# argumentcomputer/lurk-beta

Measured on NVIDIA H100. Metric: Lurk iterations proved/sec (fib rc=100, Nova IVC), higher is better.
Workload: dtype u32x8 (254-bit Montgomery integers)

## Files before the change

lurk-beta_b200/csrc/foldctx_impl.cuh:

```cuda
#pragma once
#include "msm_impl.cuh"
#include "poseidon_api.h"
#include "trie.cuh"
#include "spmv3.cuh"

#include <memory>
#include <string>

namespace lurk {

static constexpr int FOLD_MAX_WORLD = 16;
static constexpr int FOLD_MAX_DEPTH = 4;
static constexpr int FOLD_MAX_SPANS = 4;
static constexpr int FOLD_RO_RATE = 24;
static constexpr int FOLD_W_WINDOW = 16;
static constexpr int FOLD_T_WINDOW = 16;

template <class F>
__global__ void __launch_bounds__(256) cross_term_dev_kernel(const F *__restrict__ az1, const F *__restrict__ bz1, const F *__restrict__ cz1,
                                                             const F *__restrict__ az2, const F *__restrict__ bz2, const F *__restrict__ cz2,
                                                             const F *__restrict__ u1p, const F *__restrict__ u2p, size_t n, F *__restrict__ t) {
    const F u1 = load_fe<F>(u1p), u2 = load_fe<F>(u2p);
    for (size_t i = (size_t)blockIdx.x * blockDim.x + threadIdx.x; i < n; i += (size_t)gridDim.x * blockDim.x) {
        WideAcc<typename F::Params> acc;
        acc.clear();
        acc.mul_acc(load_fe<F>(az1 + i), load_fe<F>(bz2 + i));
        acc.mul_acc(load_fe<F>(az2 + i), load_fe<F>(bz1 + i));
        F pos = acc.reduce();
        WideAcc<typename F::Params> neg;
        neg.clear();
        neg.mul_acc(u1, load_fe<F>(cz2 + i));
        neg.mul_acc(u2, load_fe<F>(cz1 + i));
        store_fe(t + i, pos - neg.reduce());
    }
}

template <class F>
struct FoldAxpyArgs {
    F *dst[5];
    const F *src[5];
    size_t end[5];
};
template <class F>
__global__ void __launch_bounds__(256) fold_axpy_kernel(FoldAxpyArgs<F> a, const F *__restrict__ rp) {
    const F r = load_fe<F>(rp);
    const size_t total = a.end[4];
    for (size_t i = (size_t)blockIdx.x * blockDim.x + threadIdx.x; i < total; i += (size_t)gridDim.x * blockDim.x) {
        int v = 0;
        while (i >= a.end[v]) v++;
        const size_t j = v ? i - a.end[v - 1] : i;
        store_fe(a.dst[v] + j, load_fe<F>(a.dst[v] + j) + r * load_fe<F>(a.src[v] + j));
    }
}

template <class F>
__global__ void __launch_bounds__(256) span_to_mont_kernel(F *base, uint64_t first, uint64_t row_elems, uint64_t stride, uint64_t rows) {
    const uint64_t total = row_elems * rows;
    for (uint64_t i = (uint64_t)blockIdx.x * blockDim.x + threadIdx.x; i < total; i += (uint64_t)gridDim.x * blockDim.x) {
        F *p = base + first + (i / row_elems) * stride + (i % row_elems);
        store_fe(p, F::from_canonical(load_fe<F>(p)));
    }
// ... 357 lines not shown
```

lurk-beta_b200/csrc/foldctx_inst.cu:

```cuda
#include "foldctx_impl.cuh"
#include "sha256.cuh"

#include <cuda.h>
#include <cstring>

namespace lurk {
LURK_MSM_EXTERN(LURK_C)
#define LURK_FOLD_POSEIDON_EXTERN(F)                                                                          \
    extern template int launch_poseidon<F, true>(int, const void *, size_t, void *, int, int, cudaStream_t, const uint64_t *, const PoseidonGather *); \
    extern template int poseidon_instance_info<F>(int, const PoseidonParams<F> **, PoseidonLayout *);        \
    extern template int launch_bitdecomp<F>(const void *, size_t, void *, int, int, cudaStream_t, const uint64_t *); \
    extern template size_t sha256_block_len<F>(int);                                                          \
    extern template int launch_sha256_witness<F>(const void *, size_t, int, void *, const uint64_t *, int, int, cudaStream_t); \
    extern template size_t trie_block_len<F>(int, int);                                                       \
    extern template int launch_trie_witness<F>(int, int, const void *, size_t, void *, const uint64_t *, int, int, cudaStream_t);
LURK_FOLD_POSEIDON_EXTERN(Fe<Bn254Fr>)
LURK_FOLD_POSEIDON_EXTERN(Fe<Bn254Fq>)
LURK_FOLD_POSEIDON_EXTERN(Fe<PallasFq>)
LURK_FOLD_POSEIDON_EXTERN(Fe<PallasFp>)

static inline int fold_grid(size_t n, int block, int per_sm) {
    size_t want = (n + block - 1) / block;
    size_t cap = (size_t)sm_count() * per_sm;
    return (int)(want < cap ? (want ? want : 1) : cap);
// ... 11 lines not shown
}

template <class C>
struct FoldCtx final : FoldCtxBase {
    using Fb = typename C::Base;
    using Fs = typename C::Scalar;
    using Pt = XYZZ<Fb>;
    using Rec = FoldRecord<Fb, Fs>;

    FoldConfigHost cfg;
    int field_id = 0;
    size_t nz = 0;
    int D = 2;
    lurk_msm_ctx *ckW[FOLD_MAX_DEPTH] = {nullptr, nullptr, nullptr, nullptr};
    lurk_msm_ctx *ckT = nullptr, *ckChk = nullptr, *ckChkW = nullptr, *ckWbase = nullptr;
    DevBuf z1, e1, T, mv1[3], z2[FOLD_MAX_DEPTH], mv2[FOLD_MAX_DEPTH][3];
    DevBuf csr_rp[3], csr_col[3], csr_val[3];
    CsrDev csr[3];
    DevBuf ro_img, step_consts[FOLD_MAX_DEPTH], r_dev, seq_dev, rec_dev[FOLD_MAX_DEPTH + 1], run_pts, xchg, bad_dev, dummy_w, dummy_p;
    bool dummy_ready = false;
    Rec *h_rec[FOLD_MAX_DEPTH + 1] = {nullptr, nullptr, nullptr, nullptr, nullptr};
    void *h_glue[FOLD_MAX_DEPTH] = {nullptr, nullptr, nullptr, nullptr};
    void *h_x2[FOLD_MAX_DEPTH] = {nullptr, nullptr, nullptr, nullptr};
    void *h_ro[FOLD_MAX_DEPTH] = {nullptr, nullptr, nullptr, nullptr};
    size_t glue_elems = 0;
    std::vector<std::unique_ptr<FoldSlotBatch>> batches;
    std::vector<FoldSpan> spans;
    PoseidonLayout roL{};
    Fb io_tag;
    int n_absorb = 0, challenge_bits = 128;
    unsigned char kinds[FOLD_RO_RATE];
    XchgBuf<Fb> *peers[FOLD_MAX_WORLD];
    bool peers_open[FOLD_MAX_WORLD];
    bool peers_set = false;
    cudaStream_t sH = nullptr, sK[3] = {nullptr, nullptr, nullptr}, sA = nullptr, sB = nullptr, sC = nullptr, sT = nullptr;
    bool partitioned = false;
    cudaEvent_t ev_h2d[FOLD_MAX_DEPTH], ev_slot[FOLD_MAX_DEPTH][3], ev_cw[FOLD_MAX_DEPTH], ev_A[FOLD_MAX_DEPTH], ev_fold[FOLD_MAX_DEPTH],
        ev_chal[FOLD_MAX_DEPTH + 1], ev_done[FOLD_MAX_DEPTH + 1];
    bool fold_recorded[FOLD_MAX_DEPTH] = {false, false, false, false};
    bool a_recorded[FOLD_MAX_DEPTH] = {false, false, false, false};
    bool b_pending[FOLD_MAX_DEPTH + 1] = {false, false, false, false, false};
    bool running_set = false;
    bool mv1_valid = false;
    unsigned launches_a = 0, launches_b = 0;
    int device = 0;
    void *green[2] = {nullptr, nullptr};
    int partition_sms[2] = {0, 0};

    FoldCtx() {
        for (int p = 0; p < FOLD_MAX_WORLD; p++) { peers[p] = nullptr; peers_open[p] = false; }
        for (int b = 0; b < FOLD_MAX_DEPTH; b++) {
            ev_h2d[b] = ev_cw[b] = ev_A[b] = ev_fold[b] = nullptr;
            for (int k = 0; k < 3; k++) ev_slot[b][k] = nullptr;
        }
        for (int b = 0; b <= FOLD_MAX_DEPTH; b++) ev_chal[b] = ev_done[b] = nullptr;
        memset(kinds, 0, sizeof kinds);
    }

    ~FoldCtx() override {
        cudaDeviceSynchronize();
        for (int p = 0; p < FOLD_MAX_WORLD; p++)
            if (peers_open[p]) cudaIpcCloseMemHandle(peers[p]);
        for (int b = 0; b < FOLD_MAX_DEPTH; b++) {
            if (ckW[b]) lurk_msm_ctx_destroy(ckW[b]);
            if (h_glue[b]) cudaFreeHost(h_glue[b]);
            if (h_x2[b]) cudaFreeHost(h_x2[b]);
            if (h_ro[b]) cudaFreeHost(h_ro[b]);
            for (cudaEvent_t e : {ev_h2d[b], ev_cw[b], ev_A[b], ev_fold[b], ev_slot[b][0], ev_slot[b][1], ev_slot[b][2]})
                if (e) cudaEventDestroy(e);
        }
        for (int b = 0; b <= FOLD_MAX_DEPTH; b++) {
            if (h_rec[b]) cudaFreeHost(h_rec[b]);
            if (ev_chal[b]) cudaEventDestroy(ev_chal[b]);
            if (ev_done[b]) cudaEventDestroy(ev_done[b]);
        }
        if (ckT) lurk_msm_ctx_destroy(ckT);
        if (ckChk) lurk_msm_ctx_destroy(ckChk);
        if (ckChkW) lurk_msm_ctx_destroy(ckChkW);
        if (ckWbase) lurk_msm_ctx_destroy(ckWbase);
        for (auto &sb : batches)
            for (int b = 0; b < FOLD_MAX_DEPTH; b++)
                if (sb->h_pre[b]) cudaFreeHost(sb->h_pre[b]);
        for (cudaStream_t s : {sH, sK[0], sK[1], sK[2], sA, sB, sC, partitioned ? sT : (cudaStream_t) nullptr})
            if (s) cudaStreamDestroy(s);
        green_destroy();
    }

    template <class Fn>
    static bool drv(const char *name, Fn *out) {
        void *p = nullptr;
        cudaDriverEntryPointQueryResult q;
        if (cudaGetDriverEntryPoint(name, &p, cudaEnableDefault, &q) != cudaSuccess || q != cudaDriverEntryPointSuccess || !p) {
            cudaGetLastError();
            return false;
        }
        *out = reinterpret_cast<Fn>(p);
        return true;
    }
    void green_destroy() {
        typedef CUresult (*destroy_t)(CUgreenCtx);
        destroy_t fn = nullptr;
        if ((green[0] || green[1]) && drv("cuGreenCtxDestroy", &fn))
            for (void *g : green)
                if (g) fn((CUgreenCtx)g);
        green[0] = green[1] = nullptr;
    }
    int green_streams(int tiny_sms, cudaStream_t *tiny, int n_tiny, cudaStream_t *big_hi, cudaStream_t *big_lo, int n_lo) {
        typedef CUresult (*get_res_t)(CUdevice, CUdevResource *, CUdevResourceType);
        typedef CUresult (*split_t)(CUdevResource *, unsigned *, const CUdevResource *, CUdevResource *, unsigned, unsigned);
        typedef CUresult (*gen_desc_t)(CUdevResourceDesc *, CUdevResource *, unsigned);
        typedef CUresult (*green_create_t)(CUgreenCtx *, CUdevResourceDesc, CUdevice, unsigned);
        typedef CUresult (*green_stream_t)(CUstream *, CUgreenCtx, unsigned, int);
        get_res_t get_res; split_t split; gen_desc_t gen_desc; green_create_t green_create; green_stream_t green_stream;
        if (!drv("cuDeviceGetDevResource", &get_res) || !drv("cuDevSmResourceSplitByCount", &split) ||
            !drv("cuDevResourceGenerateDesc", &gen_desc) || !drv("cuGreenCtxCreate", &green_create) ||
            !drv("cuGreenCtxStreamCreate", &green_stream))
            return LURK_ERR_CUDA;
        CUdevResource all, part, rest;
        if (get_res((CUdevice)device, &all, CU_DEV_RESOURCE_TYPE_SM)) return LURK_ERR_CUDA;
        unsigned groups = 1;
        if (split(&part, &groups, &all, &rest, 0, (unsigned)tiny_sms) || groups != 1) return LURK_ERR_CUDA;
        CUdevResourceDesc desc[2] = {nullptr, nullptr};
        if (gen_desc(&desc[0], &part, 1) || gen_desc(&desc[1], &rest, 1)) return LURK_ERR_CUDA;
        if (green_create((CUgreenCtx *)&green[0], desc[0], (CUdevice)device, CU_GREEN_CTX_DEFAULT_STREAM) ||
            green_create((CUgreenCtx *)&green[1], desc[1], (CUdevice)device, CU_GREEN_CTX_DEFAULT_STREAM)) { green_destroy(); return LURK_ERR_CUDA; }
        partition_sms[0] = (int)part.sm.smCount;
        partition_sms[1] = (int)rest.sm.smCount;
        int rc = 0;
        for (int k = 0; k < n_tiny; k++) rc |= green_stream((CUstream *)(tiny + k), (CUgreenCtx)green[0], CU_STREAM_NON_BLOCKING, -1);
        rc |= green_stream((CUstream *)big_hi, (CUgreenCtx)green[1], CU_STREAM_NON_BLOCKING, -1);
        for (int k = 0; k < n_lo; k++) rc |= green_stream((CUstream *)(big_lo + k), (CUgreenCtx)green[1], CU_STREAM_NON_BLOCKING, 0);
        if (rc) { green_destroy(); return LURK_ERR_CUDA; }
        return LURK_OK;
    }

    int init(const FoldConfigHost &c, const uint64_t *const row_ptr[3], const uint32_t *const col[3], const uint8_t *const val[3], int fmt,
             lurk_msm_ctx *ck_w, lurk_msm_ctx *ck_t) override {
        cfg = c;
        D = c.depth;
        nz = (size_t)c.n_w + 1 + (size_t)c.n_x;
        field_id = C::ID == 0 ? LURK_FIELD_BN254_FR : C::ID == 1 ? LURK_FIELD_BN254_FQ : C::ID == 2 ? LURK_FIELD_PALLAS_FQ : LURK_FIELD_PALLAS_FP;
        LURK_CUDA_TRY(cudaGetDevice(&device));
        if (ck_w->curve_id != C::ID || ck_t->curve_id != C::ID) { set_error("commitment key belongs to another curve"); return LURK_ERR_ARG; }
        if (ck_w->n < c.n_w || ck_t->n < c.n_rows) { set_error("commitment key shorter than the witness / the constraint count"); return LURK_ERR_ARG; }
        if (ck_w->device != device || ck_t->device != device) { set_error("commitment key lives on another device"); return LURK_ERR_ARG; }
// ... 20 lines not shown
                ckT->n = c.n_rows;
                ckT->d_table = nullptr;
                ckT->owns_table = false;
                ckT->fixed_c = 0;
                LURK_TRY(msm_precompute<C>(ckT, want));
            }
        }
        LURK_TRY(lurk_msm_ctx_clone(ck_t, &ckChk));
        LURK_TRY(lurk_msm_ctx_clone(ck_w, &ckChkW));
        for (int b = 0; b < D; b++) lurk_msm_ctx_set_profiling(ckW[b], 1);
        lurk_msm_ctx_set_profiling(ckT, 1);

        int lo = 0, hi = 0;
        LURK_CUDA_TRY(cudaDeviceGetStreamPriorityRange(&lo, &hi));
        if (c.latency_sms > 0) {
            cudaStream_t tiny[2] = {nullptr, nullptr}, big_lo[4] = {nullptr, nullptr, nullptr, nullptr};
            if (green_streams(c.latency_sms, tiny, 2, &sB, big_lo, 4) != LURK_OK) {
                set_error("SM partitioning (green contexts) is not available on this driver");
                return LURK_ERR_CUDA;
            }
            sT = tiny[0]; sC = tiny[1];
            sK[0] = big_lo[0]; sK[1] = big_lo[1]; sK[2] = big_lo[2]; sA = big_lo[3];
            partitioned = true;
        } else {
            LURK_CUDA_TRY(cudaStreamCreateWithPriority(&sB, cudaStreamNonBlocking, hi));
            for (int k = 0; k < 3; k++) LURK_CUDA_TRY(cudaStreamCreateWithPriority(&sK[k], cudaStreamNonBlocking, lo));
            LURK_CUDA_TRY(cudaStreamCreateWithPriority(&sA, cudaStreamNonBlocking, lo));
            LURK_CUDA_TRY(cudaStreamCreateWithPriority(&sC, cudaStreamNonBlocking, lo));
            sT = sB;
        }
        LURK_CUDA_TRY(cudaStreamCreateWithPriority(&sH, cudaStreamNonBlocking, lo));
        if (partitioned) {
            for (lurk_msm_ctx *m : {ckW[0], ckW[1], ckW[2], ckW[3], ckT, ckChk, ckChkW}) {
                if (!m) continue;
                m->tiny_stream = sT;
                LURK_CUDA_TRY(cudaEventCreateWithFlags(&m->ev_fork, cudaEventDisableTiming));
                LURK_CUDA_TRY(cudaEventCreateWithFlags(&m->ev_join, cudaEventDisableTiming));
            }
        }
        auto mkev = [](cudaEvent_t *e) { return cudaEventCreateWithFlags(e, cudaEventDisableTiming); };
        for (int b = 0; b < D; b++) {
            LURK_CUDA_TRY(mkev(&ev_h2d[b])); LURK_CUDA_TRY(mkev(&ev_cw[b])); LURK_CUDA_TRY(mkev(&ev_A[b])); LURK_CUDA_TRY(mkev(&ev_fold[b]));
            for (int k = 0; k < 3; k++) LURK_CUDA_TRY(mkev(&ev_slot[b][k]));
        }
        for (int b = 0; b <= D; b++) { LURK_CUDA_TRY(mkev(&ev_chal[b])); LURK_CUDA_TRY(mkev(&ev_done[b])); }

        LURK_TRY(z1.alloc(nz * sizeof(Fs)));
        LURK_TRY(e1.alloc((size_t)c.n_rows * sizeof(Fs)));
        LURK_TRY(T.alloc((size_t)c.n_rows * sizeof(Fs)));
        for (int m = 0; m < 3; m++) LURK_TRY(mv1[m].alloc((size_t)c.n_rows * sizeof(Fs)));
        const Fs one = Fs::one();
        for (int b = 0; b < D; b++) {
            LURK_TRY(z2[b].alloc(nz * sizeof(Fs)));
            LURK_CUDA_TRY(cudaMemset(z2[b].p, 0, nz * sizeof(Fs)));
            LURK_CUDA_TRY(cudaMemcpy(z2[b].as<Fs>() + c.n_w, &one, sizeof(Fs), cudaMemcpyHostToDevice));
            for (int m = 0; m < 3; m++) LURK_TRY(mv2[b][m].alloc((size_t)c.n_rows * sizeof(Fs)));
            LURK_TRY(step_consts[b].alloc(FOLD_RO_RATE * sizeof(Fb)));
            LURK_CUDA_TRY(cudaMemset(step_consts[b].p, 0, FOLD_RO_RATE * sizeof(Fb)));
            LURK_CUDA_TRY(cudaMallocHost(&h_ro[b], FOLD_RO_RATE * 32));
            memset(h_ro[b], 0, FOLD_RO_RATE * 32);
            if (c.n_x) { LURK_CUDA_TRY(cudaMallocHost(&h_x2[b], (size_t)c.n_x * 32)); memset(h_x2[b], 0, (size_t)c.n_x * 32); }
        }
        LURK_CUDA_TRY(cudaMemset(z1.p, 0, nz * sizeof(Fs)));
        LURK_CUDA_TRY(cudaMemset(e1.p, 0, (size_t)c.n_rows * sizeof(Fs)));
        for (int b = 0; b <= D; b++) {
            LURK_TRY(rec_dev[b].alloc(sizeof(Rec)));
            LURK_CUDA_TRY(cudaMemset(rec_dev[b].p, 0, sizeof(Rec)));
            LURK_CUDA_TRY(cudaMallocHost((void **)&h_rec[b], sizeof(Rec)));
            memset(h_rec[b], 0, sizeof(Rec));
        }
        LURK_TRY(r_dev.alloc(sizeof(Fs)));
        LURK_TRY(seq_dev.alloc(sizeof(unsigned long long)));
        LURK_CUDA_TRY(cudaMemset(seq_dev.p, 0, sizeof(unsigned long long)));
        LURK_TRY(run_pts.alloc(2 * sizeof(Pt)));
        LURK_CUDA_TRY(cudaMemset(run_pts.p, 0, 2 * sizeof(Pt)));
        LURK_TRY(bad_dev.alloc(sizeof(SatCount)));
        LURK_TRY(xchg.alloc(sizeof(XchgBuf<Fb>)));
        LURK_CUDA_TRY(cudaMemset(xchg.p, 0, sizeof(XchgBuf<Fb>)));
        peers[c.rank] = xchg.as<XchgBuf<Fb>>();

        for (int m = 0; m < 3; m++) {
            const size_t nnz = c.n_rows ? (size_t)row_ptr[m][c.n_rows] : 0;
            for (size_t k = 0; k < nnz; k++)
                if (col[m][k] >= nz) { set_error("matrix %d: column %u out of range", m, col[m][k]); return LURK_ERR_ARG; }
            LURK_TRY(csr_rp[m].alloc(((size_t)c.n_rows + 1) * sizeof(uint64_t)));
            LURK_TRY(csr_col[m].alloc(std::max<size_t>(1, nnz) * sizeof(uint32_t)));
// ... 124 lines not shown
        else if (which == FOLD_BUF_RO) { p = h_ro[b]; n = FOLD_RO_RATE * 32; }
        else { set_error("no host buffer %d", which); return LURK_ERR_ARG; }
        if (ptr) *ptr = p;
        if (bytes) *bytes = n;
        return LURK_OK;
    }
    int device_buffer(int b, int which, void **ptr, size_t *bytes) override {
        void *p = nullptr;
        size_t n = 0;
        if (which >= 0) {
            LURK_TRY(chk_b(b));
            if (which >= (int)batches.size()) { set_error("no slot batch %d", which); return LURK_ERR_ARG; }
            p = batches[which]->d_pre[b].p; n = batches[which]->bytes();
        } else if (which == FOLD_BUF_W2) { LURK_TRY(chk_b(b)); p = z2[b].p; n = nz * 32; }
        else if (which == FOLD_BUF_RO) { LURK_TRY(chk_b(b)); p = step_consts[b].p; n = FOLD_RO_RATE * 32; }
        else if (which == FOLD_BUF_T) { p = T.p; n = (size_t)cfg.n_rows * 32; }
        else if (which == FOLD_BUF_Z1) { p = z1.p; n = nz * 32; }
        else if (which == FOLD_BUF_E1) { p = e1.p; n = (size_t)cfg.n_rows * 32; }
        else { set_error("no device buffer %d", which); return LURK_ERR_ARG; }
        if (ptr) *ptr = p;
        if (bytes) *bytes = n;
        return LURK_OK;
    }

    int exchange_handle(uint8_t out[64]) override {
        static_assert(sizeof(cudaIpcMemHandle_t) == 64, "handle size");
        cudaIpcMemHandle_t h;
        LURK_CUDA_TRY(cudaIpcGetMemHandle(&h, xchg.p));
        memcpy(out, &h, 64);
        return LURK_OK;
    }
    int set_peers(const uint8_t *handles) override {
        if (cfg.world <= 1) return LURK_OK;
// ... 28 lines not shown
        *out = Pt::from_affine(a);
        return LURK_OK;
    }

    int upload_vec(void *dst, const uint8_t *src, size_t n, int fmt) {
        if (!n) return LURK_OK;
        LURK_CUDA_TRY(cudaMemcpyAsync(dst, src, n * 32, cudaMemcpyHostToDevice, sB));
        int bad = 0;
        LURK_TRY(check_reduced_dev<Fs>(dst, n, sB, &bad));
        if (bad) { set_error("%d element(s) not reduced below the field modulus", bad); return LURK_ERR_RANGE; }
        if (fmt == LURK_FMT_CANONICAL) LURK_TRY(convert_dev<Fs>(dst, n, LURK_FMT_MONTGOMERY, dst, sB));
        return LURK_OK;
    }
    int set_running(const uint8_t *w, const uint8_t *e, const uint8_t *u, const uint8_t *x, const uint8_t *comm_w, const uint8_t *comm_e,
                    int fmt) override {
        LURK_TRY(sync());
        LURK_TRY(upload_vec(z1.p, w, cfg.n_w, fmt));
        LURK_TRY(upload_vec(z1.as<Fs>() + cfg.n_w, u, 1, fmt));
        LURK_TRY(upload_vec(z1.as<Fs>() + cfg.n_w + 1, x, cfg.n_x, fmt));
        LURK_TRY(upload_vec(e1.p, e, cfg.n_rows, fmt));
        Pt pts[2];
        LURK_TRY(point_from_bytes(comm_w, fmt, &pts[0]));
        LURK_TRY(point_from_bytes(comm_e, fmt, &pts[1]));
        LURK_CUDA_TRY(cudaMemcpyAsync(run_pts.p, pts, sizeof pts, cudaMemcpyHostToDevice, sB));
        LURK_CUDA_TRY(cudaStreamSynchronize(sB));
        running_set = true;
        mv1_valid = false;
        return LURK_OK;
    }
    int download_vec(uint8_t *dst, const void *src, size_t n, int fmt) {
        if (!n || !dst) return LURK_OK;
        if (fmt == LURK_FMT_MONTGOMERY) {
            LURK_CUDA_TRY(cudaMemcpyAsync(dst, src, n * 32, cudaMemcpyDeviceToHost, sB));
        } else {
            void *tmp = nullptr;
            LURK_CUDA_TRY(cudaMallocAsync(&tmp, n * 32, sB));
            int rc = convert_dev<Fs>(src, n, LURK_FMT_CANONICAL, tmp, sB);
            cudaError_t e = cudaMemcpyAsync(dst, tmp, n * 32, cudaMemcpyDeviceToHost, sB);
            cudaFreeAsync(tmp, sB);
            LURK_TRY(rc);
            LURK_CUDA_TRY(e);
        }
        return LURK_OK;
    }
    int get_running(uint8_t *w, uint8_t *e, uint8_t *u, uint8_t *x, uint8_t *comm_w, uint8_t *comm_e, int fmt) override {
        LURK_TRY(sync());
        LURK_TRY(download_vec(w, z1.p, cfg.n_w, fmt));
        LURK_TRY(download_vec(u, z1.as<Fs>() + cfg.n_w, 1, fmt));
        LURK_TRY(download_vec(x, z1.as<Fs>() + cfg.n_w + 1, cfg.n_x, fmt));
        LURK_TRY(download_vec(e, e1.p, cfg.n_rows, fmt));
        Pt pts[2];
        LURK_CUDA_TRY(cudaMemcpyAsync(pts, run_pts.p, sizeof pts, cudaMemcpyDeviceToHost, sB));
        LURK_CUDA_TRY(cudaStreamSynchronize(sB));
        if (comm_w) point_to_bytes(pts[0], fmt, comm_w);
        if (comm_e) point_to_bytes(pts[1], fmt, comm_e);
        return LURK_OK;
    }

    int prepare_dummy() {
        if (dummy_ready) return LURK_OK;
// ... 29 lines not shown
        LURK_TRY(dummy_p.alloc(64));
        LURK_CUDA_TRY(cudaMemcpy(dummy_p.p, pt, 64, cudaMemcpyHostToDevice));
        for (int k = 0; k < D; k++) { ckW[k]->d_sub = dummy_w.p; ckW[k]->d_offset = dummy_p.p; }
        return LURK_OK;
    }

    int stage_a(int b, int flags, int fmt) override {
        LURK_TRY(chk_b(b));
        LURK_TRY(prepare_dummy());
        if (fmt != LURK_FMT_CANONICAL && fmt != LURK_FMT_MONTGOMERY) { set_error("bad format %d", fmt); return LURK_ERR_ARG; }
        if (b_pending[b]) { set_error("buffer %d: the previous step's result has not been collected", b); return LURK_ERR_ARG; }
        const bool staged = !(flags & FOLD_INPUTS_RESIDENT);
        static const bool skip_a = getenv("LURK_FOLD_SKIP_STAGE_A") != nullptr;
        if (skip_a && !staged && a_recorded[b]) return LURK_OK;
        if (!staged && fmt != LURK_FMT_MONTGOMERY) { set_error("device-resident inputs are Montgomery form"); return LURK_ERR_ARG; }
        Fs *W2 = z2[b].as<Fs>();
        unsigned k = 0;
        if (fold_recorded[b]) LURK_CUDA_TRY(cudaStreamWaitEvent(sH, ev_fold[b], 0));
        if (staged) {
            for (auto &sb : batches)
                if (sb->count) LURK_CUDA_TRY(cudaMemcpyAsync(sb->d_pre[b].p, sb->h_pre[b], sb->bytes(), cudaMemcpyHostToDevice, sH));
            size_t off = 0;
            for (const FoldSpan &s : spans) {
                LURK_CUDA_TRY(cudaMemcpy2DAsync(W2 + s.first, s.stride * 32, (const uint8_t *)h_glue[b] + off * 32, s.row_elems * 32, s.row_elems * 32,
                                                s.rows, cudaMemcpyHostToDevice, sH));
                if (fmt == LURK_FMT_CANONICAL) {
                    span_to_mont_kernel<Fs><<<fold_grid(s.rows * s.row_elems, 256, 4), 256, 0, sH>>>(W2, s.first, s.row_elems, s.stride, s.rows);
                    k++;
                }
                off += s.rows * s.row_elems;
            }
            if (cfg.n_x) {
                LURK_CUDA_TRY(cudaMemcpyAsync(W2 + cfg.n_w + 1, h_x2[b], (size_t)cfg.n_x * 32, cudaMemcpyHostToDevice, sH));
// ... 19 lines not shown
            } else if (sb->arity) {
                LURK_TRY((launch_poseidon<Fs, true>(sb->arity, sb->d_pre[b].p, sb->count, W2, fmt, LURK_FMT_MONTGOMERY, st, sb->d_offsets.as<uint64_t>())));
            } else {
                uint32_t mod[8];
                for (int i = 0; i < 8; i++) mod[i] = Fs::Params::MOD(i);
                LURK_TRY(bitdecomp_fold(sb->d_pre[b].p, sb->count, W2, bitdecomp_block_host(mod), fmt, st, sb->d_offsets.as<uint64_t>()));
            }
            k++;
        }
        for (int s = 0; s < 3; s++) LURK_CUDA_TRY(cudaEventRecord(ev_slot[b][s], sK[s]));
        for (int s = 1; s < 3; s++) LURK_CUDA_TRY(cudaStreamWaitEvent(sK[0], ev_slot[b][s], 0));
        LURK_TRY(msm_launch<C>(ckW[b], W2, cfg.n_w, LURK_FMT_MONTGOMERY, sK[0], false));
        k += ckW[b]->last_launches;
        LURK_CUDA_TRY(cudaEventRecord(ev_cw[b], partitioned ? sT : sK[0]));
        for (int s = 0; s < 3; s++) LURK_CUDA_TRY(cudaStreamWaitEvent(sA, ev_slot[b][s], 0));
        if (cfg.n_rows) {
            spmv3_kernel<Fs><<<dim3(fold_grid(cfg.n_rows, 256, 8), 3), 256, 0, sA>>>(csr[0], csr[1], csr[2], cfg.n_rows, z2[b].as<Fs>(), mv2[b][0].as<Fs>(),
                                                                                    mv2[b][1].as<Fs>(), mv2[b][2].as<Fs>());
            k++;
        }
        LURK_CUDA_TRY(cudaGetLastError());
        LURK_CUDA_TRY(cudaEventRecord(ev_A[b], sA));
        a_recorded[b] = true;
        launches_a = k;
        return LURK_OK;
    }

    int bitdecomp_fold(const void *d_vals, size_t n, void *d_base, int blk, int fmt, cudaStream_t st, const uint64_t *d_offs) {
        if (fmt == LURK_FMT_MONTGOMERY) return launch_bitdecomp<Fs>(d_vals, n, d_base, blk, LURK_FMT_MONTGOMERY, st, d_offs);
        LURK_TRY(convert_dev<Fs>(d_vals, n, LURK_FMT_MONTGOMERY, const_cast<void *>(d_vals), st));
// ... 16 lines not shown
        a.mode = mode;
        a.r_out = r_dev.as<Fs>();
        a.rec = rec_dev[rec_index].as<Rec>();
        return a;
    }
    int need_peers() const {
        if (cfg.world > 1 && !peers_set) { set_error("sharded key: call lurk_fold_ctx_set_peers before the first step"); return LURK_ERR_ARG; }
        return LURK_OK;
    }

    int init_running(int b) override {
        LURK_TRY(chk_b(b));
        LURK_TRY(need_peers());
        if (!a_recorded[b]) { set_error("buffer %d: stage A has not been enqueued", b); return LURK_ERR_ARG; }
        if (b_pending[b]) { set_error("buffer %d: result not collected", b); return LURK_ERR_ARG; }
        LURK_CUDA_TRY(cudaStreamWaitEvent(sB, ev_A[b], 0));
        LURK_CUDA_TRY(cudaMemcpyAsync(z1.p, z2[b].p, nz * sizeof(Fs), cudaMemcpyDeviceToDevice, sB));
        LURK_CUDA_TRY(cudaMemsetAsync(e1.p, 0, (size_t)cfg.n_rows * sizeof(Fs), sB));
        for (int m = 0; m < 3 && cfg.n_rows; m++)
            LURK_CUDA_TRY(cudaMemcpyAsync(mv1[m].p, mv2[b][m].p, (size_t)cfg.n_rows * sizeof(Fs), cudaMemcpyDeviceToDevice, sB));
        mv1_valid = true;
        LURK_CUDA_TRY(cudaStreamWaitEvent(sT, ev_cw[b], 0));
        fold_challenge_kernel<C><<<1, 64, 0, sT>>>(challenge_args(ckW[b]->scratch.result.template as<Pt>(), nullptr, b, b, FOLD_MODE_COMMIT_ONLY));
        LURK_CUDA_TRY(cudaGetLastError());
        LURK_CUDA_TRY(cudaEventRecord(ev_chal[b], sT));
        if (sT != sB) LURK_CUDA_TRY(cudaStreamWaitEvent(sB, ev_chal[b], 0));
        LURK_CUDA_TRY(cudaEventRecord(ev_fold[b], sB));
        fold_recorded[b] = true;
        LURK_CUDA_TRY(cudaStreamWaitEvent(sC, ev_chal[b], 0));
        fold_commitments_kernel<C><<<1, 64, 0, sC>>>(run_pts.as<Pt>(), run_pts.as<Pt>() + 1, rec_dev[b].as<Rec>(), 1);
        LURK_CUDA_TRY(cudaGetLastError());
        LURK_CUDA_TRY(cudaMemcpyAsync(h_rec[b], rec_dev[b].p, sizeof(Rec), cudaMemcpyDeviceToHost, sC));
        LURK_CUDA_TRY(cudaEventRecord(ev_done[b], sC));
        b_pending[b] = true;
        running_set = true;
        launches_b = 2;
        return LURK_OK;
    }

    int stage_b_launch(int b) override {
        LURK_TRY(chk_b(b));
        LURK_TRY(need_peers());
        if (!running_set) { set_error("no running instance (lurk_fold_ctx_init_running or _set_running first)"); return LURK_ERR_ARG; }
        if (!a_recorded[b]) { set_error("buffer %d: stage A has not been enqueued", b); return LURK_ERR_ARG; }
        if (b_pending[b]) { set_error("buffer %d: the previous step's result has not been collected", b); return LURK_ERR_ARG; }
        unsigned k = 0;
        const size_t rows = cfg.n_rows;
        if (rows && !mv1_valid) {
            spmv3_kernel<Fs><<<dim3(fold_grid(rows, 256, 8), 3), 256, 0, sB>>>(csr[0], csr[1], csr[2], rows, z1.as<Fs>(), mv1[0].as<Fs>(), mv1[1].as<Fs>(),
                                                                             mv1[2].as<Fs>());
            k++;
        }
        mv1_valid = true;
        LURK_CUDA_TRY(cudaStreamWaitEvent(sB, ev_A[b], 0));
        if (rows) {
            cross_term_dev_kernel<Fs><<<fold_grid(rows, 256, 8), 256, 0, sB>>>(mv1[0].as<Fs>(), mv1[1].as<Fs>(), mv1[2].as<Fs>(), mv2[b][0].as<Fs>(),
                                                                              mv2[b][1].as<Fs>(), mv2[b][2].as<Fs>(), z1.as<Fs>() + cfg.n_w,
                                                                              z2[b].as<Fs>() + cfg.n_w, rows, T.as<Fs>());
            k++;
        }
        LURK_TRY(msm_launch<C>(ckT, T.p, rows, LURK_FMT_MONTGOMERY, sB, false));
        k += rows ? ckT->last_launches : 0;
        if (sT != sB && !rows) {
            LURK_CUDA_TRY(cudaEventRecord(ev_chal[b], sB));
            LURK_CUDA_TRY(cudaStreamWaitEvent(sT, ev_chal[b], 0));
        }
        LURK_CUDA_TRY(cudaStreamWaitEvent(sT, ev_cw[b], 0));
        fold_challenge_kernel<C><<<1, 64, 0, sT>>>(challenge_args(ckW[b]->scratch.result.template as<Pt>(), ckT->scratch.result.template as<Pt>(), b, b,
                                                                  FOLD_MODE_FOLD));
        k++;
        LURK_CUDA_TRY(cudaEventRecord(ev_chal[b], sT));
        if (sT != sB) LURK_CUDA_TRY(cudaStreamWaitEvent(sB, ev_chal[b], 0));
        {
            FoldAxpyArgs<Fs> ax;
            ax.dst[0] = z1.as<Fs>(); ax.src[0] = z2[b].as<Fs>(); ax.end[0] = nz;
            ax.dst[1] = e1.as<Fs>(); ax.src[1] = T.as<Fs>(); ax.end[1] = nz + rows;
            for (int m = 0; m < 3; m++) { ax.dst[2 + m] = mv1[m].as<Fs>(); ax.src[2 + m] = mv2[b][m].as<Fs>(); ax.end[2 + m] = nz + (size_t)(2 + m) * rows; }
            fold_axpy_kernel<Fs><<<fold_grid(ax.end[4], 256, 8), 256, 0, sB>>>(ax, r_dev.as<Fs>());
            k++;
        }
        LURK_CUDA_TRY(cudaGetLastError());
        LURK_CUDA_TRY(cudaEventRecord(ev_fold[b], sB));
        fold_recorded[b] = true;
        LURK_CUDA_TRY(cudaStreamWaitEvent(sC, ev_chal[b], 0));
        fold_commitments_kernel<C><<<1, 64, 0, sC>>>(run_pts.as<Pt>(), run_pts.as<Pt>() + 1, rec_dev[b].as<Rec>(), 0);
        k++;
        LURK_CUDA_TRY(cudaGetLastError());
        LURK_CUDA_TRY(cudaMemcpyAsync(h_rec[b], rec_dev[b].p, sizeof(Rec), cudaMemcpyDeviceToHost, sC));
        LURK_CUDA_TRY(cudaEventRecord(ev_done[b], sC));
        b_pending[b] = true;
        launches_b = k;
        return LURK_OK;
    }

    int collect(int b, FoldResultHost *out, int fmt) override {
        LURK_TRY(chk_b(b));
        if (!b_pending[b]) { set_error("buffer %d: nothing to collect", b); return LURK_ERR_ARG; }
        LURK_CUDA_TRY(cudaEventSynchronize(ev_done[b]));
        b_pending[b] = false;
        const Rec &r = *h_rec[b];
        if (out) {
            point_bytes(r.cw_x, r.cw_y, r.cw_inf, fmt, out->comm_w);
            point_bytes(r.ct_x, r.ct_y, r.ct_inf, fmt, out->comm_t);
            point_bytes(r.uw_x, r.uw_y, r.uw_inf, fmt, out->run_comm_w);
            point_bytes(r.ue_x, r.ue_y, r.ue_inf, fmt, out->run_comm_e);
            Fs rr = fmt == LURK_FMT_CANONICAL ? r.r.to_canonical() : r.r;
            memcpy(out->r, rr.v, 32);
            Fb hh = fmt == LURK_FMT_CANONICAL ? r.hash.to_canonical() : r.hash;
            memcpy(out->hash, hh.v, 32);
            out->status = (int)r.status;
            out->seq = r.seq;
        }
        if (r.status) { set_error("partial-commitment exchange timed out (a peer rank did not reach step %llu)", r.seq); return LURK_ERR_CUDA; }
        return LURK_OK;
    }

    int check_running(unsigned long long *bad_rows, int *comm_w_ok, int *comm_e_ok) override {
        LURK_TRY(need_peers());
        LURK_TRY(sync());
        const size_t rows = cfg.n_rows;
        const Fs *kept[3] = {mv1[0].as<Fs>(), mv1[1].as<Fs>(), mv1[2].as<Fs>()};
        SatCount cnt{0, 0};
        LURK_TRY(r1cs_sat_launch<Fs>(csr, rows, z1.as<Fs>(), cfg.n_w, e1.as<Fs>(), mv1_valid ? kept : nullptr, bad_dev.as<SatCount>(), sB));
        LURK_CUDA_TRY(cudaMemcpyAsync(&cnt, bad_dev.p, sizeof cnt, cudaMemcpyDeviceToHost, sB));
        LURK_TRY(msm_launch<C>(ckChkW, z1.p, cfg.n_w, LURK_FMT_MONTGOMERY, sB, false));
        LURK_TRY(msm_launch<C>(ckChk, e1.p, rows, LURK_FMT_MONTGOMERY, sB, false));
        if (sT != sB) {
            LURK_CUDA_TRY(cudaEventRecord(ev_chal[D], sB));
            LURK_CUDA_TRY(cudaStreamWaitEvent(sT, ev_chal[D], 0));
        }
        fold_challenge_kernel<C><<<1, 64, 0, sT>>>(challenge_args(ckChkW->scratch.result.template as<Pt>(), ckChk->scratch.result.template as<Pt>(), 0, D,
                                                                  FOLD_MODE_COMMIT_ONLY));
        LURK_CUDA_TRY(cudaGetLastError());
// ... 15 lines not shown
        return LURK_OK;
    }

    int stats(unsigned *la, unsigned *lb, float *acc_w_ms, float *acc_t_ms) override {
        LURK_TRY(sync());
        if (la) *la = launches_a;
        if (lb) *lb = launches_b;
        float ms = 0.f;
        if (acc_w_ms) { *acc_w_ms = 0.f; if (ckW[0]->ev0 && cudaEventElapsedTime(&ms, ckW[0]->ev0, ckW[0]->ev1) == cudaSuccess) *acc_w_ms = ms; }
        if (acc_t_ms) { *acc_t_ms = 0.f; if (ckT->ev0 && cudaEventElapsedTime(&ms, ckT->ev0, ckT->ev1) == cudaSuccess) *acc_t_ms = ms; }
        cudaGetLastError();
        return LURK_OK;
    }

    int sync() override {
        for (cudaStream_t s : {sH, sK[0], sK[1], sK[2], sA, sB, sC, sT})
            if (s) LURK_CUDA_TRY(cudaStreamSynchronize(s));
        return LURK_OK;
    }
};

template <class C>
FoldCtxBase *make_fold_ctx() { return new FoldCtx<C>(); }
template FoldCtxBase *make_fold_ctx<LURK_C>();

}
```

Baseline: 25610.

## Defer mv1 fold into next cross-term kernel and move W/E fold to side stream

The running-instance fold of the three matrix-vector products (mv1 += r*mv2) is deferred and fused into the next step's cross-term kernel, which folds, stores and consumes them in one pass. u1 is carried through a small device ring. The remaining W/E axpy now runs on a new high-priority stream sW, off the critical sB path. T is double-buffered per depth slot so the next cross term can overlap. This saves a full read/write pass over mv1 and shortens the serial chain, at the cost of more complex event dependencies and flush calls on every API path that reads state.

```diff
diff --git a/lurk-beta_b200/csrc/foldctx_impl.cuh b/lurk-beta_b200/csrc/foldctx_impl.cuh
--- a/lurk-beta_b200/csrc/foldctx_impl.cuh
+++ b/lurk-beta_b200/csrc/foldctx_impl.cuh
@@ -17,21 +17,48 @@
 static constexpr int FOLD_T_WINDOW = 16;
 
 template <class F>
-__global__ void __launch_bounds__(256) cross_term_dev_kernel(const F *__restrict__ az1, const F *__restrict__ bz1, const F *__restrict__ cz1,
-                                                             const F *__restrict__ az2, const F *__restrict__ bz2, const F *__restrict__ cz2,
-                                                             const F *__restrict__ u1p, const F *__restrict__ u2p, size_t n, F *__restrict__ t) {
-    const F u1 = load_fe<F>(u1p), u2 = load_fe<F>(u2p);
-    for (size_t i = (size_t)blockIdx.x * blockDim.x + threadIdx.x; i < n; i += (size_t)gridDim.x * blockDim.x) {
+struct CrossTermArgs {
+    F *mv1[3];
+    const F *mvp[3];
+    const F *mv2[3];
+    const F *r;
+    const F *u1, *u2;
+    F *u_next;
+    size_t n;
+    F *t;
+};
+template <class F, bool FOLD>
+__global__ void __launch_bounds__(256, 3) cross_term_fold_kernel(CrossTermArgs<F> a) {
+    F u1 = load_fe<F>(a.u1), r = F::zero();
+    if (FOLD) {
+        r = load_fe<F>(a.r);
+        u1 = u1 + r * load_fe<F>(a.u1 + 1);
+    }
+    const F u2 = load_fe<F>(a.u2);
+    if (blockIdx.x == 0 && threadIdx.x == 0) { store_fe(a.u_next, u1); store_fe(a.u_next + 1, u2); }
+    for (size_t i = (size_t)blockIdx.x * blockDim.x + threadIdx.x; i < a.n; i += (size_t)gridDim.x * blockDim.x) {
         WideAcc<typename F::Params> acc;
         acc.clear();
-        acc.mul_acc(load_fe<F>(az1 + i), load_fe<F>(bz2 + i));
-        acc.mul_acc(load_fe<F>(az2 + i), load_fe<F>(bz1 + i));
-        F pos = acc.reduce();
+        {
+            F az1 = load_fe<F>(a.mv1[0] + i);
+            if (FOLD) { az1 = az1 + r * load_fe<F>(a.mvp[0] + i); store_fe(a.mv1[0] + i, az1); }
+            acc.mul_acc(az1, load_fe<F>(a.mv2[1] + i));
+        }
+        {
+            F bz1 = load_fe<F>(a.mv1[1] + i);
+            if (FOLD) { bz1 = bz1 + r * load_fe<F>(a.mvp[1] + i); store_fe(a.mv1[1] + i, bz1); }
+            acc.mul_acc(load_fe<F>(a.mv2[0] + i), bz1);
+        }
+        const F pos = acc.reduce();
         WideAcc<typename F::Params> neg;
         neg.clear();
-        neg.mul_acc(u1, load_fe<F>(cz2 + i));
-        neg.mul_acc(u2, load_fe<F>(cz1 + i));
-        store_fe(t + i, pos - neg.reduce());
+        neg.mul_acc(u1, load_fe<F>(a.mv2[2] + i));
+        {
+            F cz1 = load_fe<F>(a.mv1[2] + i);
+            if (FOLD) { cz1 = cz1 + r * load_fe<F>(a.mvp[2] + i); store_fe(a.mv1[2] + i, cz1); }
+            neg.mul_acc(u2, cz1);
+        }
+        store_fe(a.t + i, pos - neg.reduce());
     }
 }
 
@@ -40,11 +67,12 @@
     F *dst[5];
     const F *src[5];
     size_t end[5];
+    int nv;
 };
 template <class F>
 __global__ void __launch_bounds__(256) fold_axpy_kernel(FoldAxpyArgs<F> a, const F *__restrict__ rp) {
     const F r = load_fe<F>(rp);
-    const size_t total = a.end[4];
+    const size_t total = a.end[a.nv - 1];
     for (size_t i = (size_t)blockIdx.x * blockDim.x + threadIdx.x; i < total; i += (size_t)gridDim.x * blockDim.x) {
         int v = 0;
         while (i >= a.end[v]) v++;
diff --git a/lurk-beta_b200/csrc/foldctx_inst.cu b/lurk-beta_b200/csrc/foldctx_inst.cu
--- a/lurk-beta_b200/csrc/foldctx_inst.cu
+++ b/lurk-beta_b200/csrc/foldctx_inst.cu
@@ -49,10 +49,11 @@
     int D = 2;
     lurk_msm_ctx *ckW[FOLD_MAX_DEPTH] = {nullptr, nullptr, nullptr, nullptr};
     lurk_msm_ctx *ckT = nullptr, *ckChk = nullptr, *ckChkW = nullptr, *ckWbase = nullptr;
-    DevBuf z1, e1, T, mv1[3], z2[FOLD_MAX_DEPTH], mv2[FOLD_MAX_DEPTH][3];
+    DevBuf z1, e1, T[FOLD_MAX_DEPTH], mv1[3], z2[FOLD_MAX_DEPTH], mv2[FOLD_MAX_DEPTH][3];
     DevBuf csr_rp[3], csr_col[3], csr_val[3];
     CsrDev csr[3];
     DevBuf ro_img, step_consts[FOLD_MAX_DEPTH], r_dev, seq_dev, rec_dev[FOLD_MAX_DEPTH + 1], run_pts, xchg, bad_dev, dummy_w, dummy_p;
+    DevBuf u_ring;
     bool dummy_ready = false;
     Rec *h_rec[FOLD_MAX_DEPTH + 1] = {nullptr, nullptr, nullptr, nullptr, nullptr};
     void *h_glue[FOLD_MAX_DEPTH] = {nullptr, nullptr, nullptr, nullptr};
@@ -68,11 +69,15 @@
     XchgBuf<Fb> *peers[FOLD_MAX_WORLD];
     bool peers_open[FOLD_MAX_WORLD];
     bool peers_set = false;
-    cudaStream_t sH = nullptr, sK[3] = {nullptr, nullptr, nullptr}, sA = nullptr, sB = nullptr, sC = nullptr, sT = nullptr;
+    cudaStream_t sH = nullptr, sK[3] = {nullptr, nullptr, nullptr}, sA = nullptr, sB = nullptr, sC = nullptr, sT = nullptr, sW = nullptr;
     bool partitioned = false;
     cudaEvent_t ev_h2d[FOLD_MAX_DEPTH], ev_slot[FOLD_MAX_DEPTH][3], ev_cw[FOLD_MAX_DEPTH], ev_A[FOLD_MAX_DEPTH], ev_fold[FOLD_MAX_DEPTH],
-        ev_chal[FOLD_MAX_DEPTH + 1], ev_done[FOLD_MAX_DEPTH + 1];
+        ev_side[FOLD_MAX_DEPTH], ev_chal[FOLD_MAX_DEPTH + 1], ev_done[FOLD_MAX_DEPTH + 1];
     bool fold_recorded[FOLD_MAX_DEPTH] = {false, false, false, false};
+    bool side_recorded[FOLD_MAX_DEPTH] = {false, false, false, false};
+    int pending = -1;
+    int u_slot = 0;
+    int last_t = 0;
     bool a_recorded[FOLD_MAX_DEPTH] = {false, false, false, false};
     bool b_pending[FOLD_MAX_DEPTH + 1] = {false, false, false, false, false};
     bool running_set = false;
@@ -85,7 +90,7 @@
     FoldCtx() {
         for (int p = 0; p < FOLD_MAX_WORLD; p++) { peers[p] = nullptr; peers_open[p] = false; }
         for (int b = 0; b < FOLD_MAX_DEPTH; b++) {
-            ev_h2d[b] = ev_cw[b] = ev_A[b] = ev_fold[b] = nullptr;
+            ev_h2d[b] = ev_cw[b] = ev_A[b] = ev_fold[b] = ev_side[b] = nullptr;
             for (int k = 0; k < 3; k++) ev_slot[b][k] = nullptr;
         }
         for (int b = 0; b <= FOLD_MAX_DEPTH; b++) ev_chal[b] = ev_done[b] = nullptr;
@@ -101,7 +106,7 @@
             if (h_glue[b]) cudaFreeHost(h_glue[b]);
             if (h_x2[b]) cudaFreeHost(h_x2[b]);
             if (h_ro[b]) cudaFreeHost(h_ro[b]);
-            for (cudaEvent_t e : {ev_h2d[b], ev_cw[b], ev_A[b], ev_fold[b], ev_slot[b][0], ev_slot[b][1], ev_slot[b][2]})
+            for (cudaEvent_t e : {ev_h2d[b], ev_cw[b], ev_A[b], ev_fold[b], ev_side[b], ev_slot[b][0], ev_slot[b][1], ev_slot[b][2]})
                 if (e) cudaEventDestroy(e);
         }
         for (int b = 0; b <= FOLD_MAX_DEPTH; b++) {
@@ -116,7 +121,7 @@
         for (auto &sb : batches)
             for (int b = 0; b < FOLD_MAX_DEPTH; b++)
                 if (sb->h_pre[b]) cudaFreeHost(sb->h_pre[b]);
-        for (cudaStream_t s : {sH, sK[0], sK[1], sK[2], sA, sB, sC, partitioned ? sT : (cudaStream_t) nullptr})
+        for (cudaStream_t s : {sH, sK[0], sK[1], sK[2], sA, sB, sC, sW, partitioned ? sT : (cudaStream_t) nullptr})
             if (s) cudaStreamDestroy(s);
         green_destroy();
     }
@@ -140,7 +145,7 @@
                 if (g) fn((CUgreenCtx)g);
         green[0] = green[1] = nullptr;
     }
-    int green_streams(int tiny_sms, cudaStream_t *tiny, int n_tiny, cudaStream_t *big_hi, cudaStream_t *big_lo, int n_lo) {
+    int green_streams(int tiny_sms, cudaStream_t *tiny, int n_tiny, cudaStream_t *big_hi, int n_hi, cudaStream_t *big_lo, int n_lo) {
         typedef CUresult (*get_res_t)(CUdevice, CUdevResource *, CUdevResourceType);
         typedef CUresult (*split_t)(CUdevResource *, unsigned *, const CUdevResource *, CUdevResource *, unsigned, unsigned);
         typedef CUresult (*gen_desc_t)(CUdevResourceDesc *, CUdevResource *, unsigned);
@@ -163,7 +168,7 @@
         partition_sms[1] = (int)rest.sm.smCount;
         int rc = 0;
         for (int k = 0; k < n_tiny; k++) rc |= green_stream((CUstream *)(tiny + k), (CUgreenCtx)green[0], CU_STREAM_NON_BLOCKING, -1);
-        rc |= green_stream((CUstream *)big_hi, (CUgreenCtx)green[1], CU_STREAM_NON_BLOCKING, -1);
+        for (int k = 0; k < n_hi; k++) rc |= green_stream((CUstream *)(big_hi + k), (CUgreenCtx)green[1], CU_STREAM_NON_BLOCKING, -1);
         for (int k = 0; k < n_lo; k++) rc |= green_stream((CUstream *)(big_lo + k), (CUgreenCtx)green[1], CU_STREAM_NON_BLOCKING, 0);
         if (rc) { green_destroy(); return LURK_ERR_CUDA; }
         return LURK_OK;
@@ -214,12 +219,13 @@
         int lo = 0, hi = 0;
         LURK_CUDA_TRY(cudaDeviceGetStreamPriorityRange(&lo, &hi));
         if (c.latency_sms > 0) {
-            cudaStream_t tiny[2] = {nullptr, nullptr}, big_lo[4] = {nullptr, nullptr, nullptr, nullptr};
-            if (green_streams(c.latency_sms, tiny, 2, &sB, big_lo, 4) != LURK_OK) {
+            cudaStream_t tiny[2] = {nullptr, nullptr}, big_hi[2] = {nullptr, nullptr}, big_lo[4] = {nullptr, nullptr, nullptr, nullptr};
+            if (green_streams(c.latency_sms, tiny, 2, big_hi, 2, big_lo, 4) != LURK_OK) {
                 set_error("SM partitioning (green contexts) is not available on this driver");
                 return LURK_ERR_CUDA;
             }
             sT = tiny[0]; sC = tiny[1];
+            sB = big_hi[0]; sW = big_hi[1];
             sK[0] = big_lo[0]; sK[1] = big_lo[1]; sK[2] = big_lo[2]; sA = big_lo[3];
             partitioned = true;
         } else {
@@ -227,6 +233,7 @@
             for (int k = 0; k < 3; k++) LURK_CUDA_TRY(cudaStreamCreateWithPriority(&sK[k], cudaStreamNonBlocking, lo));
             LURK_CUDA_TRY(cudaStreamCreateWithPriority(&sA, cudaStreamNonBlocking, lo));
             LURK_CUDA_TRY(cudaStreamCreateWithPriority(&sC, cudaStreamNonBlocking, lo));
+            LURK_CUDA_TRY(cudaStreamCreateWithPriority(&sW, cudaStreamNonBlocking, hi));
             sT = sB;
         }
         LURK_CUDA_TRY(cudaStreamCreateWithPriority(&sH, cudaStreamNonBlocking, lo));
@@ -241,17 +248,18 @@
         auto mkev = [](cudaEvent_t *e) { return cudaEventCreateWithFlags(e, cudaEventDisableTiming); };
         for (int b = 0; b < D; b++) {
             LURK_CUDA_TRY(mkev(&ev_h2d[b])); LURK_CUDA_TRY(mkev(&ev_cw[b])); LURK_CUDA_TRY(mkev(&ev_A[b])); LURK_CUDA_TRY(mkev(&ev_fold[b]));
+            LURK_CUDA_TRY(mkev(&ev_side[b]));
             for (int k = 0; k < 3; k++) LURK_CUDA_TRY(mkev(&ev_slot[b][k]));
         }
         for (int b = 0; b <= D; b++) { LURK_CUDA_TRY(mkev(&ev_chal[b])); LURK_CUDA_TRY(mkev(&ev_done[b])); }
 
         LURK_TRY(z1.alloc(nz * sizeof(Fs)));
         LURK_TRY(e1.alloc((size_t)c.n_rows * sizeof(Fs)));
-        LURK_TRY(T.alloc((size_t)c.n_rows * sizeof(Fs)));
         for (int m = 0; m < 3; m++) LURK_TRY(mv1[m].alloc((size_t)c.n_rows * sizeof(Fs)));
         const Fs one = Fs::one();
         for (int b = 0; b < D; b++) {
             LURK_TRY(z2[b].alloc(nz * sizeof(Fs)));
+            LURK_TRY(T[b].alloc((size_t)c.n_rows * sizeof(Fs)));
             LURK_CUDA_TRY(cudaMemset(z2[b].p, 0, nz * sizeof(Fs)));
             LURK_CUDA_TRY(cudaMemcpy(z2[b].as<Fs>() + c.n_w, &one, sizeof(Fs), cudaMemcpyHostToDevice));
             for (int m = 0; m < 3; m++) LURK_TRY(mv2[b][m].alloc((size_t)c.n_rows * sizeof(Fs)));
@@ -270,6 +278,8 @@
             memset(h_rec[b], 0, sizeof(Rec));
         }
         LURK_TRY(r_dev.alloc(sizeof(Fs)));
+        LURK_TRY(u_ring.alloc(4 * sizeof(Fs)));
+        LURK_CUDA_TRY(cudaMemset(u_ring.p, 0, 4 * sizeof(Fs)));
         LURK_TRY(seq_dev.alloc(sizeof(unsigned long long)));
         LURK_CUDA_TRY(cudaMemset(seq_dev.p, 0, sizeof(unsigned long long)));
         LURK_TRY(run_pts.alloc(2 * sizeof(Pt)));
@@ -424,9 +434,13 @@
             p = batches[which]->d_pre[b].p; n = batches[which]->bytes();
         } else if (which == FOLD_BUF_W2) { LURK_TRY(chk_b(b)); p = z2[b].p; n = nz * 32; }
         else if (which == FOLD_BUF_RO) { LURK_TRY(chk_b(b)); p = step_consts[b].p; n = FOLD_RO_RATE * 32; }
-        else if (which == FOLD_BUF_T) { p = T.p; n = (size_t)cfg.n_rows * 32; }
-        else if (which == FOLD_BUF_Z1) { p = z1.p; n = nz * 32; }
-        else if (which == FOLD_BUF_E1) { p = e1.p; n = (size_t)cfg.n_rows * 32; }
+        else if (which == FOLD_BUF_T) { p = T[last_t].p; n = (size_t)cfg.n_rows * 32; }
+        else if (which == FOLD_BUF_Z1 || which == FOLD_BUF_E1) {
+            LURK_TRY(flush());
+            LURK_TRY(sync());
+            if (which == FOLD_BUF_Z1) { p = z1.p; n = nz * 32; }
+            else { p = e1.p; n = (size_t)cfg.n_rows * 32; }
+        }
         else { set_error("no device buffer %d", which); return LURK_ERR_ARG; }
         if (ptr) *ptr = p;
         if (bytes) *bytes = n;
@@ -485,6 +499,7 @@
     }
     int set_running(const uint8_t *w, const uint8_t *e, const uint8_t *u, const uint8_t *x, const uint8_t *comm_w, const uint8_t *comm_e,
                     int fmt) override {
+        LURK_TRY(flush());
         LURK_TRY(sync());
         LURK_TRY(upload_vec(z1.p, w, cfg.n_w, fmt));
         LURK_TRY(upload_vec(z1.as<Fs>() + cfg.n_w, u, 1, fmt));
@@ -515,6 +530,7 @@
         return LURK_OK;
     }
     int get_running(uint8_t *w, uint8_t *e, uint8_t *u, uint8_t *x, uint8_t *comm_w, uint8_t *comm_e, int fmt) override {
+        LURK_TRY(flush());
         LURK_TRY(sync());
         LURK_TRY(download_vec(w, z1.p, cfg.n_w, fmt));
         LURK_TRY(download_vec(u, z1.as<Fs>() + cfg.n_w, 1, fmt));
@@ -574,9 +590,10 @@
         static const bool skip_a = getenv("LURK_FOLD_SKIP_STAGE_A") != nullptr;
         if (skip_a && !staged && a_recorded[b]) return LURK_OK;
         if (!staged && fmt != LURK_FMT_MONTGOMERY) { set_error("device-resident inputs are Montgomery form"); return LURK_ERR_ARG; }
+        if (pending == b) LURK_TRY(flush());
         Fs *W2 = z2[b].as<Fs>();
         unsigned k = 0;
-        if (fold_recorded[b]) LURK_CUDA_TRY(cudaStreamWaitEvent(sH, ev_fold[b], 0));
+        if (side_recorded[b]) LURK_CUDA_TRY(cudaStreamWaitEvent(sH, ev_side[b], 0));
         if (staged) {
             for (auto &sb : batches)
                 if (sb->count) LURK_CUDA_TRY(cudaMemcpyAsync(sb->d_pre[b].p, sb->h_pre[b], sb->bytes(), cudaMemcpyHostToDevice, sH));
@@ -626,6 +643,7 @@
         k += ckW[b]->last_launches;
         LURK_CUDA_TRY(cudaEventRecord(ev_cw[b], partitioned ? sT : sK[0]));
         for (int s = 0; s < 3; s++) LURK_CUDA_TRY(cudaStreamWaitEvent(sA, ev_slot[b][s], 0));
+        if (fold_recorded[b]) LURK_CUDA_TRY(cudaStreamWaitEvent(sA, ev_fold[b], 0));
         if (cfg.n_rows) {
             spmv3_kernel<Fs><<<dim3(fold_grid(cfg.n_rows, 256, 8), 3), 256, 0, sA>>>(csr[0], csr[1], csr[2], cfg.n_rows, z2[b].as<Fs>(), mv2[b][0].as<Fs>(),
                                                                                     mv2[b][1].as<Fs>(), mv2[b][2].as<Fs>());
@@ -672,6 +690,7 @@
         LURK_TRY(need_peers());
         if (!a_recorded[b]) { set_error("buffer %d: stage A has not been enqueued", b); return LURK_ERR_ARG; }
         if (b_pending[b]) { set_error("buffer %d: result not collected", b); return LURK_ERR_ARG; }
+        LURK_TRY(flush());
         LURK_CUDA_TRY(cudaStreamWaitEvent(sB, ev_A[b], 0));
         LURK_CUDA_TRY(cudaMemcpyAsync(z1.p, z2[b].p, nz * sizeof(Fs), cudaMemcpyDeviceToDevice, sB));
         LURK_CUDA_TRY(cudaMemsetAsync(e1.p, 0, (size_t)cfg.n_rows * sizeof(Fs), sB));
@@ -684,7 +703,8 @@
         LURK_CUDA_TRY(cudaEventRecord(ev_chal[b], sT));
         if (sT != sB) LURK_CUDA_TRY(cudaStreamWaitEvent(sB, ev_chal[b], 0));
         LURK_CUDA_TRY(cudaEventRecord(ev_fold[b], sB));
-        fold_recorded[b] = true;
+        LURK_CUDA_TRY(cudaEventRecord(ev_side[b], sB));
+        fold_recorded[b] = side_recorded[b] = true;
         LURK_CUDA_TRY(cudaStreamWaitEvent(sC, ev_chal[b], 0));
         fold_commitments_kernel<C><<<1, 64, 0, sC>>>(run_pts.as<Pt>(), run_pts.as<Pt>() + 1, rec_dev[b].as<Rec>(), 1);
         LURK_CUDA_TRY(cudaGetLastError());
@@ -710,15 +730,36 @@
             k++;
         }
         mv1_valid = true;
+        if (side_recorded[b]) LURK_CUDA_TRY(cudaStreamWaitEvent(sB, ev_side[b], 0));
         LURK_CUDA_TRY(cudaStreamWaitEvent(sB, ev_A[b], 0));
+        const int pb = pending;
         if (rows) {
-            cross_term_dev_kernel<Fs><<<fold_grid(rows, 256, 8), 256, 0, sB>>>(mv1[0].as<Fs>(), mv1[1].as<Fs>(), mv1[2].as<Fs>(), mv2[b][0].as<Fs>(),
-                                                                              mv2[b][1].as<Fs>(), mv2[b][2].as<Fs>(), z1.as<Fs>() + cfg.n_w,
-                                                                              z2[b].as<Fs>() + cfg.n_w, rows, T.as<Fs>());
+            CrossTermArgs<Fs> ct;
+            Fs *ring = u_ring.as<Fs>();
+            for (int m = 0; m < 3; m++) {
+                ct.mv1[m] = mv1[m].as<Fs>();
+                ct.mvp[m] = pb >= 0 ? mv2[pb][m].as<Fs>() : nullptr;
+                ct.mv2[m] = mv2[b][m].as<Fs>();
+            }
+            ct.r = pb >= 0 ? &rec_dev[pb].as<Rec>()->r : nullptr;
+            ct.u1 = pb >= 0 ? ring + 2 * (u_slot ^ 1) : z1.as<Fs>() + cfg.n_w;
+            ct.u2 = z2[b].as<Fs>() + cfg.n_w;
+            ct.u_next = ring + 2 * u_slot;
+            ct.n = rows;
+            ct.t = T[b].as<Fs>();
+            if (pb >= 0) cross_term_fold_kernel<Fs, true><<<fold_grid(rows, 256, 8), 256, 0, sB>>>(ct);
+            else cross_term_fold_kernel<Fs, false><<<fold_grid(rows, 256, 8), 256, 0, sB>>>(ct);
             k++;
         }
-        LURK_TRY(msm_launch<C>(ckT, T.p, rows, LURK_FMT_MONTGOMERY, sB, false));
+        u_slot ^= 1;
+        if (pb >= 0) {
+            LURK_CUDA_TRY(cudaEventRecord(ev_fold[pb], sB));
+            fold_recorded[pb] = true;
+            pending = -1;
+        }
+        LURK_TRY(msm_launch<C>(ckT, T[b].p, rows, LURK_FMT_MONTGOMERY, sB, false));
         k += rows ? ckT->last_launches : 0;
+        last_t = b;
         if (sT != sB && !rows) {
             LURK_CUDA_TRY(cudaEventRecord(ev_chal[b], sB));
             LURK_CUDA_TRY(cudaStreamWaitEvent(sT, ev_chal[b], 0));
@@ -729,17 +770,19 @@
         k++;
         LURK_CUDA_TRY(cudaEventRecord(ev_chal[b], sT));
         if (sT != sB) LURK_CUDA_TRY(cudaStreamWaitEvent(sB, ev_chal[b], 0));
+        pending = b;
+        LURK_CUDA_TRY(cudaStreamWaitEvent(sW, ev_chal[b], 0));
         {
             FoldAxpyArgs<Fs> ax;
             ax.dst[0] = z1.as<Fs>(); ax.src[0] = z2[b].as<Fs>(); ax.end[0] = nz;
-            ax.dst[1] = e1.as<Fs>(); ax.src[1] = T.as<Fs>(); ax.end[1] = nz + rows;
-            for (int m = 0; m < 3; m++) { ax.dst[2 + m] = mv1[m].as<Fs>(); ax.src[2 + m] = mv2[b][m].as<Fs>(); ax.end[2 + m] = nz + (size_t)(2 + m) * rows; }
-            fold_axpy_kernel<Fs><<<fold_grid(ax.end[4], 256, 8), 256, 0, sB>>>(ax, r_dev.as<Fs>());
+            ax.dst[1] = e1.as<Fs>(); ax.src[1] = T[b].as<Fs>(); ax.end[1] = nz + rows;
+            ax.nv = 2;
+            fold_axpy_kernel<Fs><<<fold_grid(ax.end[1], 256, 8), 256, 0, sW>>>(ax, &rec_dev[b].as<Rec>()->r);
             k++;
         }
         LURK_CUDA_TRY(cudaGetLastError());
-        LURK_CUDA_TRY(cudaEventRecord(ev_fold[b], sB));
-        fold_recorded[b] = true;
+        LURK_CUDA_TRY(cudaEventRecord(ev_side[b], sW));
+        side_recorded[b] = true;
         LURK_CUDA_TRY(cudaStreamWaitEvent(sC, ev_chal[b], 0));
         fold_commitments_kernel<C><<<1, 64, 0, sC>>>(run_pts.as<Pt>(), run_pts.as<Pt>() + 1, rec_dev[b].as<Rec>(), 0);
         k++;
@@ -751,10 +794,29 @@
         return LURK_OK;
     }
 
+    int flush() {
+        if (pending < 0) return LURK_OK;
+        const int pb = pending;
+        const size_t rows = cfg.n_rows;
+        if (rows) {
+            FoldAxpyArgs<Fs> ax;
+            for (int m = 0; m < 3; m++) { ax.dst[m] = mv1[m].as<Fs>(); ax.src[m] = mv2[pb][m].as<Fs>(); ax.end[m] = (size_t)(m + 1) * rows; }
+            ax.nv = 3;
+            fold_axpy_kernel<Fs><<<fold_grid(ax.end[2], 256, 8), 256, 0, sB>>>(ax, &rec_dev[pb].as<Rec>()->r);
+            LURK_CUDA_TRY(cudaGetLastError());
+        }
+        LURK_CUDA_TRY(cudaEventRecord(ev_fold[pb], sB));
+        fold_recorded[pb] = true;
+        LURK_CUDA_TRY(cudaStreamWaitEvent(sB, ev_side[pb], 0));
+        pending = -1;
+        return LURK_OK;
+    }
+
     int collect(int b, FoldResultHost *out, int fmt) override {
         LURK_TRY(chk_b(b));
         if (!b_pending[b]) { set_error("buffer %d: nothing to collect", b); return LURK_ERR_ARG; }
         LURK_CUDA_TRY(cudaEventSynchronize(ev_done[b]));
+        if (side_recorded[b]) LURK_CUDA_TRY(cudaEventSynchronize(ev_side[b]));
         b_pending[b] = false;
         const Rec &r = *h_rec[b];
         if (out) {
@@ -775,6 +837,7 @@
 
     int check_running(unsigned long long *bad_rows, int *comm_w_ok, int *comm_e_ok) override {
         LURK_TRY(need_peers());
+        LURK_TRY(flush());
         LURK_TRY(sync());
         const size_t rows = cfg.n_rows;
         const Fs *kept[3] = {mv1[0].as<Fs>(), mv1[1].as<Fs>(), mv1[2].as<Fs>()};
@@ -820,7 +883,7 @@
     }
 
     int sync() override {
-        for (cudaStream_t s : {sH, sK[0], sK[1], sK[2], sA, sB, sC, sT})
+        for (cudaStream_t s : {sH, sK[0], sK[1], sK[2], sA, sB, sC, sT, sW})
             if (s) LURK_CUDA_TRY(cudaStreamSynchronize(s));
         return LURK_OK;
     }
```

New measurement: 25930 (median of 6 runs). No clear change (+1.2%).
